# BatsResearch/menghini-neurips23-code

Measured on AMD Instinct MI355X. Metric: images/sec CLIP ViT-B/16 encode+prompt-step, higher is better.
Workload: dtype f16

## Files before the change

### menghini-neurips23-code_amd/csrc/attention_split.hip

```cpp
#include <math.h>

#include "common.h"

__device__ __forceinline__ int vt_index_fwd_s(int key, int d) { return vt_index(key, ((d >> 2) & 3) * 16 + (d >> 4) * 4 + (d & 3)); }

__device__ __forceinline__ void split8(const f32x4 a, const f32x4 b, half8& hi, half8& lo) {
    half4 h0, l0, h1, l1;
    split_f16x4(a, h0, l0);
    split_f16x4(b, h1, l1);
    hi = (half8){h0[0], h0[1], h0[2], h0[3], h1[0], h1[1], h1[2], h1[3]};
    lo = (half8){l0[0], l0[1], l0[2], l0[3], l1[0], l1[1], l1[2], l1[3]};
}

template <int KVC, bool CAUSAL, int NW>
__global__ __launch_bounds__(NW * 64) void attn_fwd_split_kernel(const float* __restrict__ qkv, half_t* __restrict__ out, int S, int H) {
    constexpr int SP = KVC * 32;
    constexpr float LOG2E = 1.4426950408889634f;
    constexpr float INV = 1.0f / (float)GRIP_SPLIT_LO_SCALE;
    extern __shared__ __attribute__((aligned(16))) char smem[];
    half_t* Kh = (half_t*)smem;
    half_t* Kl = Kh + SP * 64;
    half_t* Vh = Kl + SP * 64;
    half_t* Vl = Vh + SP * 64;

    const int tid = threadIdx.x, lane = tid & 63, wave = tid >> 6;
    const int D = H * 64;
    const int b = blockIdx.x / H, h = blockIdx.x - b * H;
    const size_t ld = (size_t)3 * D;
    const float* base = qkv + (size_t)b * S * ld + h * 64;
    const int li = lane & 15, lg = lane >> 4;
    const int n_qt = (S + 15) >> 4;

    for (int idx = tid; idx < SP * 8; idx += NW * 64) {
        const int row = idx >> 3, chunk = idx & 7;
        f32x4 a = {0.f, 0.f, 0.f, 0.f}, c = {0.f, 0.f, 0.f, 0.f};
        if (row < S) {
            const f32x4* p = (const f32x4*)(base + (size_t)row * ld + D + chunk * 8);
            a = p[0];
            c = p[1];
        }
        half8 hi, lo;
        split8(a, c, hi, lo);
        const int o = row * 64 + ((chunk ^ (row & 7)) * 8);
        *(half8*)(Kh + o) = hi;
        *(half8*)(Kl + o) = lo;
    }
    for (int idx = tid; idx < ((SP / 2 + 31) / 32) * 256; idx += NW * 64) {
        const int lane_rp = idx & 31, chunk = ((idx >> 5) & 1) + 2 * ((idx >> 6) & 3), rblk = idx >> 8;
        const int r0 = 2 * (rblk * 32 + lane_rp);
        if (r0 >= SP) continue;
        f32x4 z = {0.f, 0.f, 0.f, 0.f};
        f32x4 a0 = z, a1 = z, b0 = z, b1 = z;
        if (r0 < S) { const f32x4* p = (const f32x4*)(base + (size_t)r0 * ld + 2 * D + chunk * 8); a0 = p[0]; a1 = p[1]; }
        if (r0 + 1 < S) { const f32x4* p = (const f32x4*)(base + (size_t)(r0 + 1) * ld + 2 * D + chunk * 8); b0 = p[0]; b1 = p[1]; }
        half8 h0, l0, h1, l1;
        split8(a0, a1, h0, l0);
        split8(b0, b1, h1, l1);
#pragma unroll
        for (int j = 0; j < 8; ++j) {
            const int o = vt_index_fwd_s(r0, chunk * 8 + j);
            *(half2v*)(Vh + o) = (half2v){h0[j], h1[j]};
            *(half2v*)(Vl + o) = (half2v){l0[j], l1[j]};
        }
    }
    __syncthreads();

    for (int qt = wave; qt < n_qt; qt += NW) {
        asm volatile("" ::: "memory");
        const int qrow = qt * 16 + li;
        const int qr = qrow < S ? qrow : S - 1;
        half8 qh[2], ql[2];
#pragma unroll
        for (int kk = 0; kk < 2; ++kk) {
            const f32x4* p = (const f32x4*)(base + (size_t)qr * ld + (kk * 4 + lg) * 8);
            split8(p[0] * 0.125f, p[1] * 0.125f, qh[kk], ql[kk]);
        }
        f32x4 sc[2 * KVC];
        float m = -INFINITY;
#pragma unroll
        for (int t = 0; t < 2 * KVC; ++t) {
            f32x4 acc = {0.f, 0.f, 0.f, 0.f}, cor = {0.f, 0.f, 0.f, 0.f};
#pragma unroll
            for (int kk = 0; kk < 2; ++kk) {
                const int o = (t * 16 + li) * 64 + (((kk * 4 + lg) ^ (lane & 7)) * 8);
                const half8 kh = *(const half8*)(Kh + o), kl = *(const half8*)(Kl + o);
                acc = __builtin_amdgcn_mfma_f32_16x16x32_f16(kh, qh[kk], acc, 0, 0, 0);
                cor = __builtin_amdgcn_mfma_f32_16x16x32_f16(kl, qh[kk], cor, 0, 0, 0);
                cor = __builtin_amdgcn_mfma_f32_16x16x32_f16(kh, ql[kk], cor, 0, 0, 0);
            }
            acc += cor * INV;
            if (CAUSAL || t >= 2 * (KVC - 1)) {
#pragma unroll
                for (int r = 0; r < 4; ++r) {
                    const int kv = t * 16 + lg * 4 + r;
                    if (kv >= S || (CAUSAL && kv > qrow)) acc[r] = -INFINITY;
                }
            }
            m = fmaxf(fmaxf(fmaxf(m, acc[0]), fmaxf(acc[1], acc[2])), acc[3]);
            sc[t] = acc;
        }
        m = fmaxf(m, __shfl_xor(m, 16));
        m = fmaxf(m, __shfl_xor(m, 32));
        const float m2 = m * LOG2E;
#pragma unroll
        for (int t = 0; t < 2 * KVC; ++t)
#pragma unroll
            for (int r = 0; r < 4; ++r) sc[t][r] = __builtin_amdgcn_exp2f(__builtin_fmaf(sc[t][r], LOG2E, -m2));

        const half8 ones = {1, 1, 1, 1, 1, 1, 1, 1};
        f32x4 sum_h = {0.f, 0.f, 0.f, 0.f}, sum_l = {0.f, 0.f, 0.f, 0.f};
        f32x4 o[4], oc[4];
#pragma unroll
        for (int nf = 0; nf < 4; ++nf) { o[nf] = (f32x4){0.f, 0.f, 0.f, 0.f}; oc[nf] = (f32x4){0.f, 0.f, 0.f, 0.f}; }
#pragma unroll
        for (int c = 0; c < KVC; ++c) {
            half8 ph, pl;
            split8(sc[2 * c], sc[2 * c + 1], ph, pl);
#pragma unroll
            for (int nf = 0; nf < 4; ++nf) {
                const int vo = (c * 4 + nf) * 512 + (lg * 16 + (li ^ lg)) * 8;
                const half8 vh = *(const half8*)(Vh + vo), vl = *(const half8*)(Vl + vo);
                o[nf] = __builtin_amdgcn_mfma_f32_16x16x32_f16(vh, ph, o[nf], 0, 0, 0);
                oc[nf] = __builtin_amdgcn_mfma_f32_16x16x32_f16(vl, ph, oc[nf], 0, 0, 0);
                oc[nf] = __builtin_amdgcn_mfma_f32_16x16x32_f16(vh, pl, oc[nf], 0, 0, 0);
            }
            sum_h = __builtin_amdgcn_mfma_f32_16x16x32_f16(ones, ph, sum_h, 0, 0, 0);
            sum_l = __builtin_amdgcn_mfma_f32_16x16x32_f16(ones, pl, sum_l, 0, 0, 0);
        }
        if (qrow < S) {
            const float inv = 1.0f / (sum_h[0] + sum_l[0] * INV);
            half_t* orow = out + (size_t)((size_t)b * S + qrow) * 2 * D;
            const int col = h * 64 + lg * 16;
            half_t* op = orow + (col >> 5) * 64 + (col & 31);
            half8 hi0, lo0, hi1, lo1;
            split8((o[0] + oc[0] * INV) * inv, (o[1] + oc[1] * INV) * inv, hi0, lo0);
            split8((o[2] + oc[2] * INV) * inv, (o[3] + oc[3] * INV) * inv, hi1, lo1);
            *(half8*)op = hi0;
            *(half8*)(op + 8) = hi1;
            *(half8*)(op + 32) = lo0;
            *(half8*)(op + 40) = lo1;
        }
    }
}

bool attention_split_supported(int S) { return S >= 1 && S <= 320; }

int launch_attention_fwd_split(const float* qkv, void* out, int B, int S, int H, int causal, hipStream_t s) {
    GRIP_REQUIRE(attention_split_supported(S) && B >= 1 && H >= 1, "attention_split: bad shape B=%d S=%d H=%d (S <= 320)", B, S, H);
    const int kvc = (S + 31) / 32;
    const size_t lds = (size_t)4 * kvc * 32 * 64 * sizeof(half_t);
#define GRIP_ATT_CASE(K)                                                                                                                     \
    case K: {                                                                                                                                \
        static bool configured = false;                                                                                                      \
        if (!configured) {                                                                                                                   \
            GRIP_CHECK_HIP(hipFuncSetAttribute((const void*)attn_fwd_split_kernel<K, false, (K >= 4 ? 8 : 4)>, hipFuncAttributeMaxDynamicSharedMemorySize, (int)lds)); \
            GRIP_CHECK_HIP(hipFuncSetAttribute((const void*)attn_fwd_split_kernel<K, true, (K >= 4 ? 8 : 4)>, hipFuncAttributeMaxDynamicSharedMemorySize, (int)lds));  \
            configured = true;                                                                                                               \
        }                                                                                                                                    \
        if (causal) hipLaunchKernelGGL((attn_fwd_split_kernel<K, true, (K >= 4 ? 8 : 4)>), dim3(B * H), dim3((K >= 4 ? 8 : 4) * 64), lds, s, qkv, (half_t*)out, S, H); \
        else hipLaunchKernelGGL((attn_fwd_split_kernel<K, false, (K >= 4 ? 8 : 4)>), dim3(B * H), dim3((K >= 4 ? 8 : 4) * 64), lds, s, qkv, (half_t*)out, S, H);       \
    } break;
    switch (kvc) {
        GRIP_ATT_CASE(1) GRIP_ATT_CASE(2) GRIP_ATT_CASE(3) GRIP_ATT_CASE(4) GRIP_ATT_CASE(5)
        GRIP_ATT_CASE(6) GRIP_ATT_CASE(7) GRIP_ATT_CASE(8) GRIP_ATT_CASE(9) GRIP_ATT_CASE(10)
        default: GRIP_REQUIRE(false, "attention_split: S = %d out of range", S);
    }
#undef GRIP_ATT_CASE
    GRIP_CHECK_HIP(hipGetLastError());
    return GRIP_OK;
}
```

Before: 21110.

## Add persistent pipelined split attention kernel prefetching next head's K/V/Q

Adds a persistent split-precision attention kernel for non-causal sequence lengths with KVC 4-7, as with ViT-B/16's 197 tokens. The grid is capped at the CU count and each block loops over (batch, head) items, loading the next item's V (and optionally K) and Q into registers while computing the current one. This hides global-load latency behind the MFMA work. It also skips the fully padded final KV tile and adds optional timestamp instrumentation behind a compile flag. The costs are higher register pressure from the prefetch buffers and fewer resident blocks than the one-block-per-head launch.

```diff
diff --git a/menghini-neurips23-code_amd/csrc/attention_split.hip b/menghini-neurips23-code_amd/csrc/attention_split.hip
--- a/menghini-neurips23-code_amd/csrc/attention_split.hip
+++ b/menghini-neurips23-code_amd/csrc/attention_split.hip
@@ -1,4 +1,5 @@
 #include <math.h>
+#include <stdlib.h>
 
 #include "common.h"
 
@@ -12,11 +13,114 @@
     lo = (half8){l0[0], l0[1], l0[2], l0[3], l1[0], l1[1], l1[2], l1[3]};
 }
 
+#ifdef GRIP_SPLIT_STAMP
+__device__ unsigned long long* grip_split_stamp_buf = nullptr;
+#define SPLIT_STAMP(slot, INSN)                                                                                                                \
+    do {                                                                                                                                       \
+        __builtin_amdgcn_sched_barrier(0);                                                                                                     \
+        unsigned long long t_;                                                                                                                 \
+        asm volatile(INSN " %0\n\ts_waitcnt lgkmcnt(0)" : "=s"(t_)::"memory");                                                                 \
+        __builtin_amdgcn_sched_barrier(0);                                                                                                     \
+        if (grip_split_stamp_buf && (threadIdx.x & 63) == 0) grip_split_stamp_buf[((size_t)blockIdx.x * NW + (threadIdx.x >> 6)) * 16 + (slot)] = t_; \
+    } while (0)
+extern "C" int grip_debug_split_attn_stamps(void* buf) {
+    GRIP_CHECK_HIP(hipMemcpyToSymbol(HIP_SYMBOL(grip_split_stamp_buf), &buf, sizeof(buf)));
+    return GRIP_OK;
+}
+#else
+#define SPLIT_STAMP(slot, INSN)
+#endif
+
+#ifndef GRIP_SPLIT_PIPE_PK
+#define GRIP_SPLIT_PIPE_PK(K) false
+#endif
+#ifndef GRIP_SPLIT_PIPE_PQ
+#define GRIP_SPLIT_PIPE_PQ(K) true
+#endif
+
+template <int KVC, bool CAUSAL, bool SKIP_DEAD>
+__device__ __forceinline__ void attn_split_tile(const half_t* Kh, const half_t* Kl, const half_t* Vh, const half_t* Vl, const half8 (&qh)[2], const half8 (&ql)[2],
+                                                int qrow, int S, half_t* obase, size_t orow_stride, int lane) {
+    constexpr float LOG2E = 1.4426950408889634f;
+    constexpr float INV = 1.0f / (float)GRIP_SPLIT_LO_SCALE;
+    const int li = lane & 15, lg = lane >> 4;
+    const bool last_dead = SKIP_DEAD && S <= (2 * KVC - 1) * 16;
+    f32x4 sc[2 * KVC];
+    float m = -INFINITY;
+#pragma unroll
+    for (int t = 0; t < 2 * KVC; ++t) {
+        if (t == 2 * KVC - 1 && last_dead) { sc[t] = (f32x4){-INFINITY, -INFINITY, -INFINITY, -INFINITY}; continue; }
+        f32x4 acc = {0.f, 0.f, 0.f, 0.f}, cor = {0.f, 0.f, 0.f, 0.f};
+#pragma unroll
+        for (int kk = 0; kk < 2; ++kk) {
+            const int o = (t * 16 + li) * 64 + (((kk * 4 + lg) ^ (lane & 7)) * 8);
+            const half8 kh = *(const half8*)(Kh + o), kl = *(const half8*)(Kl + o);
+            acc = __builtin_amdgcn_mfma_f32_16x16x32_f16(kh, qh[kk], acc, 0, 0, 0);
+            cor = __builtin_amdgcn_mfma_f32_16x16x32_f16(kl, qh[kk], cor, 0, 0, 0);
+            cor = __builtin_amdgcn_mfma_f32_16x16x32_f16(kh, ql[kk], cor, 0, 0, 0);
+        }
+        acc += cor * INV;
+        if (CAUSAL || t >= 2 * (KVC - 1)) {
+#pragma unroll
+            for (int r = 0; r < 4; ++r) {
+                const int kv = t * 16 + lg * 4 + r;
+                if (kv >= S || (CAUSAL && kv > qrow)) acc[r] = -INFINITY;
+            }
+        }
+        m = fmaxf(fmaxf(fmaxf(m, acc[0]), fmaxf(acc[1], acc[2])), acc[3]);
+        sc[t] = acc;
+    }
+    m = fmaxf(m, __shfl_xor(m, 16));
+    m = fmaxf(m, __shfl_xor(m, 32));
+    const float m2 = m * LOG2E;
+#pragma unroll
+    for (int t = 0; t < 2 * KVC; ++t) {
+        if (t == 2 * KVC - 1 && last_dead) { sc[t] = (f32x4){0.f, 0.f, 0.f, 0.f}; continue; }
+#pragma unroll
+        for (int r = 0; r < 4; ++r) sc[t][r] = __builtin_amdgcn_exp2f(__builtin_fmaf(sc[t][r], LOG2E, -m2));
+    }
+
+    const half8 ones = {1, 1, 1, 1, 1, 1, 1, 1};
+    f32x4 sum_h = {0.f, 0.f, 0.f, 0.f}, sum_l = {0.f, 0.f, 0.f, 0.f};
+    f32x4 o[4], oc[4];
+#pragma unroll
+    for (int nf = 0; nf < 4; ++nf) { o[nf] = (f32x4){0.f, 0.f, 0.f, 0.f}; oc[nf] = (f32x4){0.f, 0.f, 0.f, 0.f}; }
+#pragma unroll
+    for (int c = 0; c < KVC; ++c) {
+        half8 ph, pl;
+        split8(sc[2 * c], sc[2 * c + 1], ph, pl);
+#pragma unroll
+        for (int nf = 0; nf < 4; ++nf) {
+            const int vo = (c * 4 + nf) * 512 + (lg * 16 + (li ^ lg)) * 8;
+            const half8 vh = *(const half8*)(Vh + vo), vl = *(const half8*)(Vl + vo);
+            o[nf] = __builtin_amdgcn_mfma_f32_16x16x32_f16(vh, ph, o[nf], 0, 0, 0);
+            oc[nf] = __builtin_amdgcn_mfma_f32_16x16x32_f16(vl, ph, oc[nf], 0, 0, 0);
+            oc[nf] = __builtin_amdgcn_mfma_f32_16x16x32_f16(vh, pl, oc[nf], 0, 0, 0);
+        }
+        sum_h = __builtin_amdgcn_mfma_f32_16x16x32_f16(ones, ph, sum_h, 0, 0, 0);
+        sum_l = __builtin_amdgcn_mfma_f32_16x16x32_f16(ones, pl, sum_l, 0, 0, 0);
+    }
+    if (qrow < S) {
+        const float inv = 1.0f / (sum_h[0] + sum_l[0] * INV);
+        half_t* op = obase + (size_t)qrow * orow_stride;
+        half8 hi0, lo0, hi1, lo1;
+        split8((o[0] + oc[0] * INV) * inv, (o[1] + oc[1] * INV) * inv, hi0, lo0);
+        split8((o[2] + oc[2] * INV) * inv, (o[3] + oc[3] * INV) * inv, hi1, lo1);
+        *(half8*)op = hi0;
+        *(half8*)(op + 8) = hi1;
+        *(half8*)(op + 32) = lo0;
+        *(half8*)(op + 40) = lo1;
+    }
+}
+
+__device__ __forceinline__ half_t* split_out_base(half_t* out, int b, int h, int S, int D, int lg) {
+    const int col = h * 64 + lg * 16;
+    return out + (size_t)b * S * 2 * D + (col >> 5) * 64 + (col & 31);
+}
+
 template <int KVC, bool CAUSAL, int NW>
 __global__ __launch_bounds__(NW * 64) void attn_fwd_split_kernel(const float* __restrict__ qkv, half_t* __restrict__ out, int S, int H) {
     constexpr int SP = KVC * 32;
-    constexpr float LOG2E = 1.4426950408889634f;
-    constexpr float INV = 1.0f / (float)GRIP_SPLIT_LO_SCALE;
     extern __shared__ __attribute__((aligned(16))) char smem[];
     half_t* Kh = (half_t*)smem;
     half_t* Kl = Kh + SP * 64;
@@ -30,6 +134,8 @@
     const float* base = qkv + (size_t)b * S * ld + h * 64;
     const int li = lane & 15, lg = lane >> 4;
     const int n_qt = (S + 15) >> 4;
+    SPLIT_STAMP(8, "s_memrealtime");
+    SPLIT_STAMP(0, "s_memtime");
 
     for (int idx = tid; idx < SP * 8; idx += NW * 64) {
         const int row = idx >> 3, chunk = idx & 7;
@@ -45,6 +151,7 @@
         *(half8*)(Kh + o) = hi;
         *(half8*)(Kl + o) = lo;
     }
+    SPLIT_STAMP(1, "s_memtime");
     for (int idx = tid; idx < ((SP / 2 + 31) / 32) * 256; idx += NW * 64) {
         const int lane_rp = idx & 31, chunk = ((idx >> 5) & 1) + 2 * ((idx >> 6) & 3), rblk = idx >> 8;
         const int r0 = 2 * (rblk * 32 + lane_rp);
@@ -63,8 +170,11 @@
             *(half2v*)(Vl + o) = (half2v){l0[j], l1[j]};
         }
     }
+    SPLIT_STAMP(2, "s_memtime");
     __syncthreads();
-
+    SPLIT_STAMP(3, "s_memtime");
+
+    half_t* obase = split_out_base(out, b, h, S, D, lg);
     for (int qt = wave; qt < n_qt; qt += NW) {
         asm volatile("" ::: "memory");
         const int qrow = qt * 16 + li;
@@ -75,79 +185,212 @@
             const f32x4* p = (const f32x4*)(base + (size_t)qr * ld + (kk * 4 + lg) * 8);
             split8(p[0] * 0.125f, p[1] * 0.125f, qh[kk], ql[kk]);
         }
-        f32x4 sc[2 * KVC];
-        float m = -INFINITY;
-#pragma unroll
-        for (int t = 0; t < 2 * KVC; ++t) {
-            f32x4 acc = {0.f, 0.f, 0.f, 0.f}, cor = {0.f, 0.f, 0.f, 0.f};
-#pragma unroll
-            for (int kk = 0; kk < 2; ++kk) {
-                const int o = (t * 16 + li) * 64 + (((kk * 4 + lg) ^ (lane & 7)) * 8);
-                const half8 kh = *(const half8*)(Kh + o), kl = *(const half8*)(Kl + o);
-                acc = __builtin_amdgcn_mfma_f32_16x16x32_f16(kh, qh[kk], acc, 0, 0, 0);
-                cor = __builtin_amdgcn_mfma_f32_16x16x32_f16(kl, qh[kk], cor, 0, 0, 0);
-                cor = __builtin_amdgcn_mfma_f32_16x16x32_f16(kh, ql[kk], cor, 0, 0, 0);
+        attn_split_tile<KVC, CAUSAL, false>(Kh, Kl, Vh, Vl, qh, ql, qrow, S, obase, (size_t)2 * D, lane);
+        SPLIT_STAMP(4 + qt / NW, "s_memtime");
+    }
+    SPLIT_STAMP(9, "s_memrealtime");
+}
+
+template <int KVC, bool PK, bool PQ>
+__global__ __launch_bounds__(512) void attn_fwd_split_pipe_kernel(const float* __restrict__ qkv, half_t* __restrict__ out, int S, int H, int n_items) {
+    constexpr int NW = 8, NT = NW * 64;
+    constexpr int SP = KVC * 32;
+    constexpr int NK = (SP * 8 + NT - 1) / NT;
+    constexpr int V_UNITS = ((SP / 2 + 31) / 32) * 256;
+    constexpr int NV = (V_UNITS + NT - 1) / NT;
+    constexpr int NQ = (2 * KVC + NW - 1) / NW;
+    extern __shared__ __attribute__((aligned(16))) char smem[];
+    half_t* Kh = (half_t*)smem;
+    half_t* Kl = Kh + SP * 64;
+    half_t* Vh = Kl + SP * 64;
+    half_t* Vl = Vh + SP * 64;
+
+    const int tid = threadIdx.x, lane = tid & 63;
+    const int wave = __builtin_amdgcn_readfirstlane(tid >> 6);
+    const int D = H * 64;
+    const unsigned ld = 3u * D;
+    const int li = lane & 15, lg = lane >> 4;
+    const int n_qt = (S + 15) >> 4;
+
+    auto item_base = [&](int item) {
+        const int b = item / H, h = item - b * H;
+        return qkv + (size_t)b * S * ld + h * 64;
+    };
+    auto opaque_tid = [&]() {
+        int t = tid;
+        asm volatile("" : "+v"(t));
+        return t;
+    };
+    f32x4 ka[NK], kc[NK];
+    auto load_k = [&](const float* base) {
+        const int t0 = opaque_tid();
+#pragma unroll
+        for (int n = 0; n < NK; ++n) {
+            const int idx = t0 + n * NT;
+            const int row = idx >> 3, chunk = idx & 7;
+            ka[n] = (f32x4){0.f, 0.f, 0.f, 0.f};
+            kc[n] = (f32x4){0.f, 0.f, 0.f, 0.f};
+            if (row < S) {
+                const f32x4* p = (const f32x4*)(base + (row * ld + D + chunk * 8));
+                ka[n] = p[0];
+                kc[n] = p[1];
             }
-            acc += cor * INV;
-            if (CAUSAL || t >= 2 * (KVC - 1)) {
-#pragma unroll
-                for (int r = 0; r < 4; ++r) {
-                    const int kv = t * 16 + lg * 4 + r;
-                    if (kv >= S || (CAUSAL && kv > qrow)) acc[r] = -INFINITY;
+        }
+    };
+    auto store_k = [&]() {
+        const int t0 = opaque_tid();
+#pragma unroll
+        for (int n = 0; n < NK; ++n) {
+            const int idx = t0 + n * NT;
+            const int row = idx >> 3, chunk = idx & 7;
+            if (idx < SP * 8) {
+                half8 hi, lo;
+                split8(ka[n], kc[n], hi, lo);
+                const int o = row * 64 + ((chunk ^ (row & 7)) * 8);
+                *(half8*)(Kh + o) = hi;
+                *(half8*)(Kl + o) = lo;
+            }
+        }
+    };
+    f32x4 va0[NV], va1[NV], vb0[NV], vb1[NV];
+    auto load_v = [&](const float* base) {
+        const int t0 = opaque_tid();
+#pragma unroll
+        for (int n = 0; n < NV; ++n) {
+            const int idx = t0 + n * NT;
+            const int lane_rp = idx & 31, chunk = ((idx >> 5) & 1) + 2 * ((idx >> 6) & 3), rblk = idx >> 8;
+            const int r0 = 2 * (rblk * 32 + lane_rp);
+            const f32x4 z = {0.f, 0.f, 0.f, 0.f};
+            va0[n] = z; va1[n] = z; vb0[n] = z; vb1[n] = z;
+            if (r0 < S) { const f32x4* p = (const f32x4*)(base + (r0 * ld + 2 * D + chunk * 8)); va0[n] = p[0]; va1[n] = p[1]; }
+            if (r0 + 1 < S) { const f32x4* p = (const f32x4*)(base + ((r0 + 1) * ld + 2 * D + chunk * 8)); vb0[n] = p[0]; vb1[n] = p[1]; }
+        }
+    };
+    auto store_v = [&]() {
+        const int t0 = opaque_tid();
+#pragma unroll
+        for (int n = 0; n < NV; ++n) {
+            const int idx = t0 + n * NT;
+            const int lane_rp = idx & 31, chunk = ((idx >> 5) & 1) + 2 * ((idx >> 6) & 3), rblk = idx >> 8;
+            const int r0 = 2 * (rblk * 32 + lane_rp);
+            if (r0 < SP) {
+                half8 h0, l0, h1, l1;
+                split8(va0[n], va1[n], h0, l0);
+                split8(vb0[n], vb1[n], h1, l1);
+#pragma unroll
+                for (int j = 0; j < 8; ++j) {
+                    const int o = vt_index_fwd_s(r0, chunk * 8 + j);
+                    *(half2v*)(Vh + o) = (half2v){h0[j], h1[j]};
+                    *(half2v*)(Vl + o) = (half2v){l0[j], l1[j]};
                 }
             }
-            m = fmaxf(fmaxf(fmaxf(m, acc[0]), fmaxf(acc[1], acc[2])), acc[3]);
-            sc[t] = acc;
-        }
-        m = fmaxf(m, __shfl_xor(m, 16));
-        m = fmaxf(m, __shfl_xor(m, 32));
-        const float m2 = m * LOG2E;
-#pragma unroll
-        for (int t = 0; t < 2 * KVC; ++t)
-#pragma unroll
-            for (int r = 0; r < 4; ++r) sc[t][r] = __builtin_amdgcn_exp2f(__builtin_fmaf(sc[t][r], LOG2E, -m2));
-
-        const half8 ones = {1, 1, 1, 1, 1, 1, 1, 1};
-        f32x4 sum_h = {0.f, 0.f, 0.f, 0.f}, sum_l = {0.f, 0.f, 0.f, 0.f};
-        f32x4 o[4], oc[4];
-#pragma unroll
-        for (int nf = 0; nf < 4; ++nf) { o[nf] = (f32x4){0.f, 0.f, 0.f, 0.f}; oc[nf] = (f32x4){0.f, 0.f, 0.f, 0.f}; }
-#pragma unroll
-        for (int c = 0; c < KVC; ++c) {
-            half8 ph, pl;
-            split8(sc[2 * c], sc[2 * c + 1], ph, pl);
-#pragma unroll
-            for (int nf = 0; nf < 4; ++nf) {
-                const int vo = (c * 4 + nf) * 512 + (lg * 16 + (li ^ lg)) * 8;
-                const half8 vh = *(const half8*)(Vh + vo), vl = *(const half8*)(Vl + vo);
-                o[nf] = __builtin_amdgcn_mfma_f32_16x16x32_f16(vh, ph, o[nf], 0, 0, 0);
-                oc[nf] = __builtin_amdgcn_mfma_f32_16x16x32_f16(vl, ph, oc[nf], 0, 0, 0);
-                oc[nf] = __builtin_amdgcn_mfma_f32_16x16x32_f16(vh, pl, oc[nf], 0, 0, 0);
+        }
+    };
+    f32x4 q0[2], q1[2];
+    auto load_q = [&](const float* base, int n) {
+        const int qrow = (wave + n * NW) * 16 + li;
+        const int qr = qrow < S ? qrow : S - 1;
+#pragma unroll
+        for (int kk = 0; kk < 2; ++kk) {
+            const f32x4* p = (const f32x4*)(base + (qr * ld + (kk * 4 + lg) * 8));
+            q0[kk] = p[0];
+            q1[kk] = p[1];
+        }
+    };
+
+    int item = blockIdx.x;
+    if (item >= n_items) return;
+    {
+        const float* base = item_base(item);
+        load_k(base);
+        load_v(base);
+        if (PQ && wave < n_qt) load_q(base, 0);
+        asm volatile("" ::: "memory");
+        store_k();
+        store_v();
+    }
+    for (;;) {
+        asm volatile("s_waitcnt lgkmcnt(0)" ::: "memory");
+        __builtin_amdgcn_s_barrier();
+        asm volatile("" ::: "memory");
+        const int next = item + gridDim.x;
+        const bool has_next = next < n_items;
+        const float* cb = item_base(item);
+        const float* nb = item_base(has_next ? next : item);
+        if (has_next) {
+            if (PK) load_k(nb);
+            load_v(nb);
+        }
+        asm volatile("" ::: "memory");
+        const int b = item / H, h = item - b * H;
+        half_t* obase = split_out_base(out, b, h, S, D, lg);
+#pragma unroll
+        for (int n = 0; n < NQ; ++n) {
+            const int qt = wave + n * NW;
+            if (qt < n_qt) {
+                asm volatile("" ::: "memory");
+                half8 qh[2], ql[2];
+                if (!PQ) load_q(cb, n);
+#pragma unroll
+                for (int kk = 0; kk < 2; ++kk) split8(q0[kk] * 0.125f, q1[kk] * 0.125f, qh[kk], ql[kk]);
+                if (PQ) {
+                    if (n + 1 < NQ && qt + NW < n_qt) load_q(cb, n + 1);
+                    else if (has_next) load_q(nb, 0);
+                }
+                asm volatile("" ::: "memory");
+                attn_split_tile<KVC, false, true>(Kh, Kl, Vh, Vl, qh, ql, qt * 16 + li, S, obase, (size_t)2 * D, lane);
             }
-            sum_h = __builtin_amdgcn_mfma_f32_16x16x32_f16(ones, ph, sum_h, 0, 0, 0);
-            sum_l = __builtin_amdgcn_mfma_f32_16x16x32_f16(ones, pl, sum_l, 0, 0, 0);
-        }
-        if (qrow < S) {
-            const float inv = 1.0f / (sum_h[0] + sum_l[0] * INV);
-            half_t* orow = out + (size_t)((size_t)b * S + qrow) * 2 * D;
-            const int col = h * 64 + lg * 16;
-            half_t* op = orow + (col >> 5) * 64 + (col & 31);
-            half8 hi0, lo0, hi1, lo1;
-            split8((o[0] + oc[0] * INV) * inv, (o[1] + oc[1] * INV) * inv, hi0, lo0);
-            split8((o[2] + oc[2] * INV) * inv, (o[3] + oc[3] * INV) * inv, hi1, lo1);
-            *(half8*)op = hi0;
-            *(half8*)(op + 8) = hi1;
-            *(half8*)(op + 32) = lo0;
-            *(half8*)(op + 40) = lo1;
-        }
+        }
+        if (!has_next) break;
+        asm volatile("s_waitcnt lgkmcnt(0)" ::: "memory");
+        __builtin_amdgcn_s_barrier();
+        asm volatile("" ::: "memory");
+        if (!PK) {
+            load_k(nb);
+            asm volatile("" ::: "memory");
+        }
+        store_k();
+        store_v();
+        item = next;
     }
 }
 
 bool attention_split_supported(int S) { return S >= 1 && S <= 320; }
+
+template <int KVC>
+static int launch_split_pipe(const float* qkv, half_t* out, int B, int S, int H, hipStream_t s) {
+    constexpr size_t lds = (size_t)4 * KVC * 32 * 64 * sizeof(half_t);
+    constexpr bool PK = GRIP_SPLIT_PIPE_PK(KVC), PQ = GRIP_SPLIT_PIPE_PQ(KVC);
+    static int n_cu = 0;
+    if (!n_cu) {
+        GRIP_CHECK_HIP(hipFuncSetAttribute((const void*)attn_fwd_split_pipe_kernel<KVC, PK, PQ>, hipFuncAttributeMaxDynamicSharedMemorySize, (int)lds));
+        int dev = 0, cus = 0;
+        GRIP_CHECK_HIP(hipGetDevice(&dev));
+        GRIP_CHECK_HIP(hipDeviceGetAttribute(&cus, hipDeviceAttributeMultiprocessorCount, dev));
+        GRIP_REQUIRE(cus >= 1, "attention_split: no compute units reported");
+        n_cu = cus;
+    }
+    const int n_items = B * H;
+    const int width = (grip_cu_budget() > 0 && grip_cu_budget() < n_cu) ? grip_cu_budget() : n_cu;
+    const int grid = n_items < width ? n_items : width;
+    hipLaunchKernelGGL((attn_fwd_split_pipe_kernel<KVC, PK, PQ>), dim3(grid), dim3(512), lds, s, qkv, out, S, H, n_items);
+    GRIP_CHECK_HIP(hipGetLastError());
+    return GRIP_OK;
+}
 
 int launch_attention_fwd_split(const float* qkv, void* out, int B, int S, int H, int causal, hipStream_t s) {
     GRIP_REQUIRE(attention_split_supported(S) && B >= 1 && H >= 1, "attention_split: bad shape B=%d S=%d H=%d (S <= 320)", B, S, H);
     const int kvc = (S + 31) / 32;
+    static const bool pipe = !(getenv("GRIP_SPLIT_ATTN_PIPE") && atoi(getenv("GRIP_SPLIT_ATTN_PIPE")) == 0);
+    if (!causal && pipe) {
+        switch (kvc) {
+            case 4: return launch_split_pipe<4>(qkv, (half_t*)out, B, S, H, s);
+            case 5: return launch_split_pipe<5>(qkv, (half_t*)out, B, S, H, s);
+            case 6: return launch_split_pipe<6>(qkv, (half_t*)out, B, S, H, s);
+            case 7: return launch_split_pipe<7>(qkv, (half_t*)out, B, S, H, s);
+            default: break;
+        }
+    }
     const size_t lds = (size_t)4 * kvc * 32 * 64 * sizeof(half_t);
 #define GRIP_ATT_CASE(K)                                                                                                                     \
     case K: {                                                                                                                                \
```

Measured after the change: 21190, median of 4. About the same (+0.4%).
